# freshman97/LinTransUNet

Hardware: AMD Instinct MI355X
Metric: 128^3 CT patches/sec (fwd+bwd) (higher is better)
Workload: dtype bf16; 1 GPU; MaskTransUnet train step (fwd + 5-level loss + bwd), 128^3 single-channel patches, 2 per GPU, dropout 0.3, random-init weights; global_batch=2, parallelism=dp1, side_stream_concurrent=True, allreduce=none (1 rank)

## Files before the change

lintransunet_amd/csrc/linattn.hip:

```cpp
#include "common.h"

#define DK 32
#define TOK 32
#define PART_STRIDE (64 + 1024)
#ifndef LA_TR_PAD
#define LA_TR_PAD 32
#endif

__device__ __forceinline__ float xhalf_sum(float v) { return xhalf_combine<LtuAdd>(v); }
__device__ __forceinline__ float xhalf_max(float v) { return xhalf_combine<LtuMax>(v); }

__device__ __forceinline__ bf16x8 pack8(const float* v) {
  bf16x8 r;
#pragma unroll
  for (int e = 0; e < 8; ++e) r[e] = (__bf16)v[e];
  return r;
}
template <typename T>
struct IsBf16 { static constexpr bool value = false; };
template <>
struct IsBf16<bf16_t> { static constexpr bool value = true; };

template <typename T>
struct GVec;
// ... 401 lines not shown
      const float4 v = *reinterpret_cast<const float4*>(qrow + 4 * q4);
      a[4 * q4] = v.x; a[4 * q4 + 1] = v.y; a[4 * q4 + 2] = v.z; a[4 * q4 + 3] = v.w;
    }
    float mx = -INFINITY;
#pragma unroll
    for (int s = 0; s < 16; ++s) mx = fmaxf(mx, a[s]);
    mx = xhalf_max(mx);
    float sum = 0.f;
#pragma unroll
    for (int s = 0; s < 16; ++s) {
      a[s] = __expf(a[s] - mx);
      sum += a[s];
    }
    sum = xhalf_sum(sum);
    const float inv = rs / sum;
    if (lh == 0 && n0 + li < n_end) {
      float* qs = qstat + (((long long)b * N + n0 + li) * H + wave) * 2;
      qs[0] = mx;
      qs[1] = inv;
    }
    f32x16 acc;
#pragma unroll
    for (int r = 0; r < 16; ++r) acc[r] = 0.f;
    if constexpr (IsBf16<T>::value) {
#pragma unroll
      for (int s = 0; s < 16; ++s) a[s] *= inv;
      acc = __builtin_amdgcn_mfma_f32_32x32x16_bf16(pack8(a), cbb[0], acc, 0, 0, 0);
      acc = __builtin_amdgcn_mfma_f32_32x32x16_bf16(pack8(a + 8), cbb[1], acc, 0, 0, 0);
    } else {
#pragma unroll
      for (int s = 0; s < 16; ++s) acc = __builtin_amdgcn_mfma_f32_32x32x2f32(a[s] * inv, cb[s], acc, 0, 0, 0);
    }
    __syncthreads();
#pragma unroll
    for (int r = 0; r < 16; ++r) {
      const int t = (r & 3) + 8 * (r >> 2) + 4 * lh;
      smem[t * LDQ + wave * DK + li] = acc[r];
    }
    __syncthreads();
    constexpr int VPR = D / W;
#pragma unroll
    for (int p = 0; p < (TOK * VPR + NTHR - 1) / NTHR; ++p) {
      const int idx = tid + p * NTHR;
      const int t = idx / VPR, c = (idx % VPR) * W;
      if (idx < TOK * VPR && n0 + t < n_end) GVec<T>::from_lds(out + ((long long)b * N + n0 + t) * D + c, &smem[t * LDQ + c]);
    }
  }
}

#define LAW_HEADS 4
#define LAW_LD (LAW_HEADS * DK + 8)

template <int D>
__global__ void __launch_bounds__(256) linattn_apply_rows(const uint16_t* __restrict__ qkv, const float* __restrict__ ctx,
                                                         uint16_t* __restrict__ out, float* __restrict__ qstat, int N, int tiles_per_wave) {
  constexpr int H = D / DK, CG = H / LAW_HEADS;
  __shared__ __attribute__((aligned(16))) uint16_t smem[4 * TOK * LAW_LD];
  const int lane = threadIdx.x & 63, wave = threadIdx.x >> 6;
  const int li = lane & 31, lh = lane >> 5;
  uint16_t* tile = smem + wave * TOK * LAW_LD;
  const int b = blockIdx.y;
  const int gw = blockIdx.x * 4 + wave;
  const int cg = gw % CG;
  const int n_begin = (gw / CG) * tiles_per_wave * TOK;
  const int n_end = min(N, n_begin + tiles_per_wave * TOK);
  if (n_begin >= N) return;
  bf16x8 ca[LAW_HEADS][2];
#pragma unroll
  for (int hh = 0; hh < LAW_HEADS; ++hh) {
    const float* cx = ctx + ((long long)b * H + cg * LAW_HEADS + hh) * 1024;
#pragma unroll
    for (int u = 0; u < 2; ++u) {
      float t[8];
#pragma unroll
      for (int e = 0; e < 8; ++e) t[e] = cx[(16 * lh + 8 * u + e) * 32 + li];
      ca[hh][u] = pack8(t);
    }
  }
  const float rs = 0.17677669529663688110f;
  const int cr = lane >> 4, cc = (lane & 15) * 8;
  const uint16_t* qb = qkv + (long long)b * N * 3 * D + cg * (LAW_HEADS * DK) + cc;
  uint16_t* ob = out + (long long)b * N * D + cg * (LAW_HEADS * DK) + cc;
  uint4 nx[8];
  auto fetch = [&](int n0) {
#pragma unroll
    for (int p = 0; p < 8; ++p) {
      const int n = n0 + 4 * p + cr;
      nx[p] = make_uint4(0u, 0u, 0u, 0u);
      if (n < n_end) nx[p] = *reinterpret_cast<const uint4*>(qb + (long long)n * 3 * D);
    }
  };
  fetch(n_begin);
  for (int n0 = n_begin; n0 < n_end; n0 += TOK) {
#pragma unroll
    for (int p = 0; p < 8; ++p) *reinterpret_cast<uint4*>(tile + (4 * p + cr) * LAW_LD + cc) = nx[p];
    if (n0 + TOK < n_end) fetch(n0 + TOK);
    float2 st[LAW_HEADS];
#pragma unroll
    for (int hh = 0; hh < LAW_HEADS; ++hh) {
      const uint16_t* qr = tile + li * LAW_LD + hh * DK + 16 * lh;
      const uint4 v0 = *reinterpret_cast<const uint4*>(qr), v1 = *reinterpret_cast<const uint4*>(qr + 8);
      const uint32_t w[8] = {v0.x, v0.y, v0.z, v0.w, v1.x, v1.y, v1.z, v1.w};
      float a[16];
#pragma unroll
      for (int k = 0; k < 8; ++k) {
        a[2 * k] = __uint_as_float(w[k] << 16);
        a[2 * k + 1] = __uint_as_float(w[k] & 0xffff0000u);
      }
      float mx = a[0];
#pragma unroll
      for (int s = 1; s < 16; ++s) mx = fmaxf(mx, a[s]);
      mx = xhalf_max(mx);
      float sum = 0.f;
#pragma unroll
      for (int s = 0; s < 16; ++s) {
        a[s] = __expf(a[s] - mx);
        sum += a[s];
      }
      sum = xhalf_sum(sum);
      const float inv = rs / sum;
      st[hh] = make_float2(mx, inv);
#pragma unroll
      for (int s = 0; s < 16; ++s) a[s] *= inv;
      f32x16 acc;
#pragma unroll
      for (int r = 0; r < 16; ++r) acc[r] = 0.f;
      acc = __builtin_amdgcn_mfma_f32_32x32x16_bf16(ca[hh][0], pack8(a), acc, 0, 0, 0);
      acc = __builtin_amdgcn_mfma_f32_32x32x16_bf16(ca[hh][1], pack8(a + 8), acc, 0, 0, 0);
#pragma unroll
      for (int q = 0; q < 4; ++q) {
        uint2 v;
        v.x = pack_bf16x2(acc[4 * q], acc[4 * q + 1]);
        v.y = pack_bf16x2(acc[4 * q + 2], acc[4 * q + 3]);
        *reinterpret_cast<uint2*>(tile + li * LAW_LD + hh * DK + 8 * q + 4 * lh) = v;
      }
    }
    if (lh == 0 && n0 + li < n_end) {
      float4* qs = reinterpret_cast<float4*>(qstat + (((long long)b * N + n0 + li) * H + cg * LAW_HEADS) * 2);
      qs[0] = make_float4(st[0].x, st[0].y, st[1].x, st[1].y);
      qs[1] = make_float4(st[2].x, st[2].y, st[3].x, st[3].y);
    }
#pragma unroll
    for (int p = 0; p < 8; ++p) {
      const int n = n0 + 4 * p + cr;
      const uint4 v = *reinterpret_cast<const uint4*>(tile + (4 * p + cr) * LAW_LD + cc);
      if (n < n_end) *reinterpret_cast<uint4*>(ob + (long long)n * D) = v;
    }
  }
}

template <typename T, int D>
__global__ void __launch_bounds__(2 * D) linattn_dctx_partial(const T* __restrict__ qkv, const T* __restrict__ dout,
                                                             const float* __restrict__ qstat, float* __restrict__ part, int N,
                                                             int tokens_per_split) {
  constexpr int H = D / DK;
  extern __shared__ __attribute__((aligned(16))) float smem[];
  float* sq = smem;
  float* sg = smem + TOK * D;
  float* st = smem + 2 * TOK * D;
  const int b = blockIdx.y, sp = blockIdx.x, nsplit = gridDim.x;
  const int tid = threadIdx.x, lane = tid & 63, wave = tid >> 6;
  const int li = lane & 31, lh = lane >> 5;
  const int n_begin = sp * tokens_per_split;
  const int n_end = min(N, n_begin + tokens_per_split);
  const T* qb = qkv + (long long)b * N * 3 * D;
  const T* gb = dout + (long long)b * N * D;
  f32x16 acc;
#pragma unroll
  for (int r = 0; r < 16; ++r) acc[r] = 0.f;
  RowTile<T, D, D, D> tq, tg;
  static_assert(TOK * H * 2 <= 2 * D, "one statistics float per thread");
  auto load_stat = [&](int n0) {
    return (tid < TOK * H * 2 && n0 + tid / (H * 2) < n_end) ? qstat[((long long)b * N + n0) * H * 2 + tid] : 0.f;
  };
  if constexpr (IsBf16<T>::value) {
    constexpr int PQ = D + LA_TR_PAD;
    uint16_t* sm = reinterpret_cast<uint16_t*>(smem);
    float* stf = reinterpret_cast<float*>(sm + 4 * TOK * PQ);
    RowTile<T, D, D, PQ> bq, bg;
    const int off = tr_lane_offset(lane, PQ) + wave * DK;
    bq.load(qb, 3 * D, 0, n_begin, n_end, tid);
    bg.load(gb, D, 0, n_begin, n_end, tid);
    float stn = load_stat(n_begin);
    bq.store_raw(sm, tid);
    bg.store_raw(sm + TOK * PQ, tid);
    if (tid < TOK * H * 2) stf[tid] = stn;
    __syncthreads();
    int buf = 0;
    for (int n0 = n_begin; n0 < n_end; n0 += TOK) {
      const bool more = n0 + TOK < n_end;
      if (more) {
        bq.load(qb, 3 * D, 0, n0 + TOK, n_end, tid);
        bg.load(gb, D, 0, n0 + TOK, n_end, tid);
        stn = load_stat(n0 + TOK);
      }
      const uint16_t* S = sm + buf * (2 * TOK * PQ);
      const float* ST = stf + buf * (TOK * H * 2);
      const int ntok = min(TOK, n_end - n0);
#pragma unroll
      for (int u = 0; u < 2; ++u) {
        const bf16x8 qf = tr_frag(S + 16 * u * PQ + off, PQ), gf = tr_frag(S + (TOK + 16 * u) * PQ + off, PQ);
        float qe[8];
#pragma unroll
        for (int e = 0; e < 8; ++e) {
          const int t = 16 * u + 8 * lh + e;
          const float2 rs = *reinterpret_cast<const float2*>(ST + (t * H + wave) * 2);
          qe[e] = t < ntok ? __expf((float)qf[e] - rs.x) * rs.y : 0.f;
        }
        acc = __builtin_amdgcn_mfma_f32_32x32x16_bf16(gf, pack8(qe), acc, 0, 0, 0);
      }
      if (more) {
        uint16_t* Sn = sm + (buf ^ 1) * (2 * TOK * PQ);
        bq.store_raw(Sn, tid);
        bg.store_raw(Sn + TOK * PQ, tid);
        if (tid < TOK * H * 2) stf[(buf ^ 1) * (TOK * H * 2) + tid] = stn;
      }
      __syncthreads();
      buf ^= 1;
    }
  } else {
  tq.load(qb, 3 * D, 0, n_begin, n_end, tid);
  tg.load(gb, D, 0, n_begin, n_end, tid);
  float stn = load_stat(n_begin);
  for (int n0 = n_begin; n0 < n_end; n0 += TOK) {
    __syncthreads();
    tq.store(sq, tid);
    tg.store(sg, tid);
    if (tid < TOK * H * 2) st[tid] = stn;
    __syncthreads();
    if (n0 + TOK < n_end) {
      tq.load(qb, 3 * D, 0, n0 + TOK, n_end, tid);
      tg.load(gb, D, 0, n0 + TOK, n_end, tid);
      stn = load_stat(n0 + TOK);
    }
    const int ntok = min(TOK, n_end - n0);
    if constexpr (IsBf16<T>::value) {
#pragma unroll
      for (int u = 0; u < 2; ++u) {
        float qe[8], ge[8];
#pragma unroll
        for (int e = 0; e < 8; ++e) {
          const int t = 16 * u + 8 * lh + e;
          qe[e] = 0.f; ge[e] = 0.f;
          if (t < ntok) {
            qe[e] = __expf(sq[t * D + wave * DK + li] - st[(t * H + wave) * 2]) * st[(t * H + wave) * 2 + 1];
            ge[e] = sg[t * D + wave * DK + li];
          }
        }
        acc = __builtin_amdgcn_mfma_f32_32x32x16_bf16(pack8(ge), pack8(qe), acc, 0, 0, 0);
      }
    } else {
#pragma unroll
      for (int t0 = 0; t0 < TOK; t0 += 2) {
        const int t = t0 + lh;
        float qv = 0.f, gv = 0.f;
        if (t < ntok) {
          qv = __expf(sq[t * D + wave * DK + li] - st[(t * H + wave) * 2]) * st[(t * H + wave) * 2 + 1];
          gv = sg[t * D + wave * DK + li];
        }
        acc = __builtin_amdgcn_mfma_f32_32x32x2f32(gv, qv, acc, 0, 0, 0);
      }
    }
  }
  }
  float* out = part + (((long long)b * nsplit + sp) * H + wave) * 1024;
#pragma unroll
  for (int r = 0; r < 16; ++r) {
    const int j = (r & 3) + 8 * (r >> 2) + 4 * lh;
    out[j * 32 + li] = acc[r];
  }
}

template <int NB>
__global__ void __launch_bounds__(256) linattn_dctx_combine(const float* __restrict__ part, float* __restrict__ dctx, int nsplit, int H) {
  __shared__ float4 red4[7][32];
  const int bh = blockIdx.y, b = bh / H, h = bh % H;
  const float* p0 = part + ((long long)b * nsplit * H + h) * 1024 + blockIdx.x * 128;
  const int l = threadIdx.x & 31, grp = threadIdx.x >> 5;
  float4 a = make_float4(0.f, 0.f, 0.f, 0.f);
  for (int s0 = grp; s0 < nsplit; s0 += 8 * NB) {
    float4 v[NB];
#pragma unroll
    for (int k = 0; k < NB; ++k) {
      const int sp = s0 + 8 * k;
      v[k] = *reinterpret_cast<const float4*>(p0 + (long long)(sp < nsplit ? sp : s0) * H * 1024 + l * 4);
    }
#pragma unroll
    for (int k = 0; k < NB; ++k)
      if (s0 + 8 * k < nsplit) { a.x += v[k].x; a.y += v[k].y; a.z += v[k].z; a.w += v[k].w; }
  }
  if (grp > 0) red4[grp - 1][l] = a;
  __syncthreads();
  if (grp != 0) return;
#pragma unroll
  for (int q = 0; q < 7; ++q) {
    const float4 v = red4[q][l];
    a.x += v.x; a.y += v.y; a.z += v.z; a.w += v.w;
  }
  const int e = blockIdx.x * 128 + l * 4, jj = e >> 5, ii = e & 31;
  float* o = dctx + (long long)bh * 1024 + jj;
  o[ii * 32] = a.x; o[(ii + 1) * 32] = a.y; o[(ii + 2) * 32] = a.z; o[(ii + 3) * 32] = a.w;
}

template <typename T, int D>
__global__ void __launch_bounds__(2 * D, 2) linattn_bwd_apply(const T* __restrict__ qkv, const T* __restrict__ dout,
                                                          const float* __restrict__ ctx, const float* __restrict__ dctx,
                                                          const float* __restrict__ stats, const float* __restrict__ tvec,
                                                          const float* __restrict__ qstat, T* __restrict__ dqkv, int N, int tokb) {
  constexpr int H = D / DK, LD3 = 3 * D + 4, LD1 = D + 4, NTHR = 2 * D, W = GVec<T>::W;
  extern __shared__ __attribute__((aligned(16))) float smem[];
  const int b = blockIdx.y;
  const int tid = threadIdx.x, lane = tid & 63, wave = tid >> 6;
  const int li = lane & 31, lh = lane >> 5;
  float* gt = smem + TOK * LD3;
  float* cs = gt + TOK * LD1 + wave * 96;
  const long long bh = (long long)b * H + wave;
  if (lane < 32) {
    cs[lane] = stats[bh * 64 + lane];
    cs[32 + lane] = 1.f / stats[bh * 64 + 32 + lane];
  }
  float ctxA[16], dcA[16], dcT[16];
#pragma unroll
  for (int s = 0; s < 16; ++s) {
    ctxA[s] = ctx[bh * 1024 + li * 32 + 16 * lh + s];
    dcA[s] = dctx[bh * 1024 + li * 32 + 16 * lh + s];
    dcT[s] = dctx[bh * 1024 + (16 * lh + s) * 32 + li];
  }
  {
    float t = 0.f;
#pragma unroll
    for (int s = 0; s < 16; ++s) t += ctxA[s] * dcA[s];
    t = xhalf_sum(t);
    if (lane < 32) cs[64 + lane] = t;
  }
  const bf16x8 ctxB[2] = {pack8(ctxA), pack8(ctxA + 8)}, dcTB[2] = {pack8(dcT), pack8(dcT + 8)};
  bf16x8 dcAB[3][2];
  {
    float r1[16], r2[16];
#pragma unroll
    for (int s = 0; s < 16; ++s) {
      r1[s] = dcA[s] - (float)(__bf16)dcA[s];
      r2[s] = r1[s] - (float)(__bf16)r1[s];
    }
#pragma unroll
    for (int u = 0; u < 2; ++u) { dcAB[0][u] = pack8(dcA + 8 * u); dcAB[1][u] = pack8(r1 + 8 * u); dcAB[2][u] = pack8(r2 + 8 * u); }
  }
  const T* qb = qkv + (long long)b * N * 3 * D;
  const T* gb = dout + (long long)b * N * D;

  const int n_begin = blockIdx.x * tokb;
  const int n_end = min(N, n_begin + tokb);
  RowTile<T, D, 3 * D, LD3> tq;
  RowTile<T, D, D, LD1> tg;
  auto load_qs = [&](int n0) {
    return *reinterpret_cast<const float2*>(qstat + (((long long)b * N + min(n0 + li, n_end - 1)) * H + wave) * 2);
  };
  tq.load(qb, 3 * D, 0, n_begin, n_end, tid);
  tg.load(gb, D, 0, n_begin, n_end, tid);
  float2 qsn = load_qs(n_begin);
  tq.store(smem, tid);
  tg.store(gt, tid);
  __syncthreads();
  for (int n0 = n_begin; n0 < n_end; n0 += TOK) {
    const float rmax = qsn.x, rinv = qsn.y;
    const bool more = n0 + TOK < n_end;
    if (more) {
      tq.load(qb, 3 * D, 0, n0 + TOK, n_end, tid);
      tg.load(gb, D, 0, n0 + TOK, n_end, tid);
      qsn = load_qs(n0 + TOK);
    }
    const float* qrow = &smem[li * LD3 + wave * DK];
    const float* krow = qrow + D;
    const float* vrow = qrow + 2 * D;
    const float* grow = &gt[li * LD1 + wave * DK];

    float gj[16], kk[16], vj[16];
#pragma unroll
    for (int q4 = 0; q4 < 4; ++q4) {
      const float4 a = *reinterpret_cast<const float4*>(grow + 16 * lh + 4 * q4);
      const float4 c = *reinterpret_cast<const float4*>(krow + 16 * lh + 4 * q4);
      const float4 e = *reinterpret_cast<const float4*>(vrow + 16 * lh + 4 * q4);
      gj[4 * q4] = a.x; gj[4 * q4 + 1] = a.y; gj[4 * q4 + 2] = a.z; gj[4 * q4 + 3] = a.w;
      kk[4 * q4] = c.x; kk[4 * q4 + 1] = c.y; kk[4 * q4 + 2] = c.z; kk[4 * q4 + 3] = c.w;
      vj[4 * q4] = e.x; vj[4 * q4 + 1] = e.y; vj[4 * q4 + 2] = e.z; vj[4 * q4 + 3] = e.w;
    }
    f32x16 aq, av, ak;
#pragma unroll
    for (int r = 0; r < 16; ++r) { aq[r] = 0.f; av[r] = 0.f; ak[r] = 0.f; }
    if constexpr (IsBf16<T>::value) {
#pragma unroll
      for (int s = 0; s < 16; ++s) kk[s] = __expf(kk[s] - cs[16 * lh + s]) * cs[32 + 16 * lh + s];
#pragma unroll
      for (int u = 0; u < 2; ++u) {
        aq = __builtin_amdgcn_mfma_f32_32x32x16_bf16(ctxB[u], pack8(gj + 8 * u), aq, 0, 0, 0);
        av = __builtin_amdgcn_mfma_f32_32x32x16_bf16(dcTB[u], pack8(kk + 8 * u), av, 0, 0, 0);
        const bf16x8 vb = pack8(vj + 8 * u);
#pragma unroll
        for (int pc = 2; pc >= 0; --pc) ak = __builtin_amdgcn_mfma_f32_32x32x16_bf16(dcAB[pc][u], vb, ak, 0, 0, 0);
      }
    } else {
#pragma unroll
      for (int s = 0; s < 16; ++s) {
        const int ch = 16 * lh + s;
        const float pk = __expf(kk[s] - cs[ch]) * cs[32 + ch];
        aq = __builtin_amdgcn_mfma_f32_32x32x2f32(ctxA[s], gj[s], aq, 0, 0, 0);
        av = __builtin_amdgcn_mfma_f32_32x32x2f32(dcT[s], pk, av, 0, 0, 0);
        ak = __builtin_amdgcn_mfma_f32_32x32x2f32(dcA[s], vj[s], ak, 0, 0, 0);
      }
    }
    float dot = 0.f;
    float qsv[16], pkv[16];
#pragma unroll
    for (int g4 = 0; g4 < 4; ++g4) {
      const int i0 = 8 * g4 + 4 * lh;
      const float4 qv = *reinterpret_cast<const float4*>(qrow + i0);
      const float4 kv = *reinterpret_cast<const float4*>(krow + i0);
      const float qa[4] = {qv.x, qv.y, qv.z, qv.w}, ka[4] = {kv.x, kv.y, kv.z, kv.w};
#pragma unroll
      for (int e = 0; e < 4; ++e) {
        const int r = 4 * g4 + e;
        qsv[r] = __expf(qa[e] - rmax) * rinv;
        pkv[r] = __expf(ka[e] - cs[i0 + e]) * cs[32 + i0 + e];
        dot += qsv[r] * aq[r];
      }
    }
    dot = xhalf_sum(dot);
    dot *= 5.65685424949238019521f;
    __syncthreads();
#pragma unroll
    for (int g4 = 0; g4 < 4; ++g4) {
      const int i0 = 8 * g4 + 4 * lh;
      float4 oq, ok4, ov;
#pragma unroll
      for (int e = 0; e < 4; ++e) {
        const int r = 4 * g4 + e;
        f4at(oq, e) = qsv[r] * (aq[r] - dot);
        f4at(ok4, e) = pkv[r] * (ak[r] - cs[64 + i0 + e]);
        f4at(ov, e) = av[r];
      }
      *reinterpret_cast<float4*>(&smem[li * LD3 + wave * DK + i0]) = oq;
      *reinterpret_cast<float4*>(&smem[li * LD3 + D + wave * DK + i0]) = ok4;
      *reinterpret_cast<float4*>(&smem[li * LD3 + 2 * D + wave * DK + i0]) = ov;
    }
    __syncthreads();
    constexpr int VPR = 3 * D / W, NOUT = (TOK * VPR + NTHR - 1) / NTHR;
    typename GVec<T>::reg ovec[NOUT];
#pragma unroll
    for (int p = 0; p < NOUT; ++p) {
      const int idx = min(tid + p * NTHR, TOK * VPR - 1);
      ovec[p] = GVec<T>::pack_lds(&smem[(idx / VPR) * LD3 + (idx % VPR) * W]);
    }
    __syncthreads();
    if (more) {
      tq.store(smem, tid);
      tg.store(gt, tid);
    }
#pragma unroll
    for (int p = 0; p < NOUT; ++p) {
      const int idx = tid + p * NTHR;
      const int t = idx / VPR, c = (idx % VPR) * W;
      if (idx < TOK * VPR && n0 + t < n_end) GVec<T>::store_g(dqkv + ((long long)b * N + n0 + t) * 3 * D + c, ovec[p]);
    }
    __syncthreads();
  }
}

static int pick_splits(int B, int N, int d, int* tokens_per_split) {
  int total = -1;
  total = ltu_knob_pos("LTU_LA_SPLITS", d >= 256 ? 256 : 512);
  int want = total / (B > 0 ? B : 1);
  if (want < 1) want = 1;
  if (want > KVC_GROUP * KVC_GROUP) want = KVC_GROUP * KVC_GROUP;
  int tps = (N + want - 1) / want;
  tps = (tps + 31) / 32 * 32;
  if (tps < 32) tps = 32;
  *tokens_per_split = tps;
  return (N + tps - 1) / tps;
}
static int pick_tokb(int B, int N, int d) {
  const int blocks = ltu_knob_pos("LTU_LA_TOKB_BLOCKS", d <= 128 ? 512 : 256);
  long long per = ((long long)B * N + blocks - 1) / blocks;
  int tokb = (int)((per + 31) / 32 * 32);
  if (tokb < 32) tokb = 32;
  if (tokb > 512) tokb = 512;
  return tokb;
}

extern "C" int ltu_linattn_splits(int B, int N) {
  int tps;
  return pick_splits(B, N, 128, &tps);
}

#define LA_DISPATCH_D(d, ...)                                   \
  do {                                                          \
    if ((d) == 32) { constexpr int D = 32; __VA_ARGS__ }        \
    else if ((d) == 64) { constexpr int D = 64; __VA_ARGS__ }   \
    else if ((d) == 128) { constexpr int D = 128; __VA_ARGS__ } \
    else if ((d) == 256) { constexpr int D = 256; __VA_ARGS__ } \
    else return LTU_E_SHAPE;                                    \
  } while (0)

extern "C" int ltu_linattn_fwd(const void* qkv, void* out, float* ctx, float* colstats, float* qstat, float* part_ws,
                               long long ws_floats, int B, int N, int d, int dtype, ltu_stream_t s);
extern "C" long long ltu_linattn_ws_floats(int B, int N, int d) {
  int tps;
  const long long ns = pick_splits(B, N, d, &tps), H = d / 32;
  return (long long)B * (ns + (ns + KVC_GROUP - 1) / KVC_GROUP + 2) * H * PART_STRIDE;
}
extern "C" int ltu_linattn_ctx(const void* qkv, float* ctx, float* colstats, float* part_ws, long long ws_floats, int B, int N, int d,
                               int dtype, ltu_stream_t s) {
  return ltu_linattn_fwd(qkv, nullptr, ctx, colstats, nullptr, part_ws, ws_floats, B, N, d, dtype, s);
}
extern "C" int ltu_linattn_fwd(const void* qkv, void* out, float* ctx, float* colstats, float* qstat, float* part_ws,
                               long long ws_floats, int B, int N, int d, int dtype, ltu_stream_t s) {
  const int H = d / 32;
  int tps;
  const int nsplit = pick_splits(B, N, d, &tps);
  if ((long long)B * (nsplit + (nsplit + KVC_GROUP - 1) / KVC_GROUP + 2) * H * PART_STRIDE > ws_floats) return LTU_E_ARG;
  hipStream_t st = (hipStream_t)s;
  const int tokb = pick_tokb(B, N, d);
  LTU_DISPATCH_T(dtype, {
    LA_DISPATCH_D(d, {
      hipLaunchKernelGGL((linattn_kv_partial<T, D>), dim3(nsplit, B), dim3(2 * D), 0, st, (const T*)qkv, part_ws, N, tps);
      const int group = KVC_GROUP, ngroups = (nsplit + group - 1) / group;
      float* part2 = part_ws + (size_t)B * nsplit * H * PART_STRIDE;
      if (nsplit * 32 * sizeof(float) <= 48 * 1024 && !ltu_knob("LTU_LA_TWO_LEVEL", 0)) {
        const size_t fsb = (size_t)nsplit * 32 * sizeof(float);
        if (nsplit <= 32) hipLaunchKernelGGL(linattn_kv_combine1<4>, dim3(8, B * H), dim3(256), fsb, st, part_ws, nsplit, colstats, ctx, H);
        else if (nsplit <= 64) hipLaunchKernelGGL(linattn_kv_combine1<8>, dim3(8, B * H), dim3(256), fsb, st, part_ws, nsplit, colstats, ctx, H);
        else if (nsplit <= 128) hipLaunchKernelGGL(linattn_kv_combine1<16>, dim3(8, B * H), dim3(256), fsb, st, part_ws, nsplit, colstats, ctx, H);
        else hipLaunchKernelGGL(linattn_kv_combine1<32>, dim3(8, B * H), dim3(256), fsb, st, part_ws, nsplit, colstats, ctx, H);
      } else if (ngroups > 1) {
        hipLaunchKernelGGL(linattn_kv_combine, dim3(ngroups, B * H), dim3(1024), 0, st, part_ws, nsplit, group, part2, colstats, ctx, H, 0);
        hipLaunchKernelGGL(linattn_kv_combine, dim3(1, B * H), dim3(1024), 0, st, part2, ngroups, ngroups, nullptr, colstats, ctx, H, 1);
      } else {
        hipLaunchKernelGGL(linattn_kv_combine, dim3(1, B * H), dim3(1024), 0, st, part_ws, nsplit, nsplit, nullptr, colstats, ctx, H, 1);
      }
      if (out == nullptr) {
      } else if constexpr (IsBf16<T>::value && D >= 128) {
        constexpr int CG = D / DK / LAW_HEADS;
        const long long tiles = cdiv(N, TOK);
        long long tpw = cdiv((long long)B * tiles * CG, (long long)ltu_knob_pos("LTU_LA_APPLY_WAVES", 4096));
        if (tpw < 1) tpw = 1;
        const long long waves = cdiv(tiles, tpw) * CG;
        hipLaunchKernelGGL((linattn_apply_rows<D>), dim3((unsigned)cdiv(waves, 4), B), dim3(256), 0, st, (const uint16_t*)qkv, ctx, (uint16_t*)out, qstat, N, (int)tpw);
      } else {
        hipLaunchKernelGGL((linattn_apply<T, D>), dim3(cdiv(N, tokb), B), dim3(2 * D), 0, st, (const T*)qkv, ctx, (T*)out, qstat, N, tokb);
      }
    });
  });
  return ltu_check_launch();
}

extern "C" int ltu_linattn_bwd(const void* qkv, const void* dout, const float* ctx, const float* colstats,
                               const float* qstat, void* dqkv, float* dctx, float* tvec, float* part_ws, long long ws_floats, int B,
                               int N, int d, int dtype, ltu_stream_t s) {
  const int H = d / 32;
  int tps;
  const int nsplit = pick_splits(B, N, d, &tps);
  if ((long long)B * nsplit * H * 1024 > ws_floats) return LTU_E_ARG;
  hipStream_t st = (hipStream_t)s;
  const size_t lds_b = (size_t)(32 * (3 * d + 4) + 32 * (d + 4) + H * 96) * sizeof(float);
  const int tokb = pick_tokb(B, N, d);
  LTU_DISPATCH_T(dtype, {
    LA_DISPATCH_D(d, {
      const size_t lds_p = IsBf16<T>::value ? (size_t)4 * TOK * (D + LA_TR_PAD) * 2 + (size_t)2 * TOK * H * 2 * sizeof(float)
                                            : (size_t)(2 * TOK * D + TOK * H * 2) * sizeof(float);
      hipLaunchKernelGGL((linattn_dctx_partial<T, D>), dim3(nsplit, B), dim3(2 * D), lds_p, st, (const T*)qkv, (const T*)dout, qstat, part_ws, N, tps);
      if (nsplit <= 32) hipLaunchKernelGGL(linattn_dctx_combine<4>, dim3(8, B * H), dim3(256), 0, st, part_ws, dctx, nsplit, H);
      else if (nsplit <= 64) hipLaunchKernelGGL(linattn_dctx_combine<8>, dim3(8, B * H), dim3(256), 0, st, part_ws, dctx, nsplit, H);
      else if (nsplit <= 128) hipLaunchKernelGGL(linattn_dctx_combine<16>, dim3(8, B * H), dim3(256), 0, st, part_ws, dctx, nsplit, H);
      else hipLaunchKernelGGL(linattn_dctx_combine<32>, dim3(8, B * H), dim3(256), 0, st, part_ws, dctx, nsplit, H);
      hipLaunchKernelGGL((linattn_bwd_apply<T, D>), dim3(cdiv(N, tokb), B), dim3(2 * D), lds_b, st, (const T*)qkv, (const T*)dout, ctx, dctx, colstats, tvec, qstat, (T*)dqkv, N, tokb);
    });
  });
  return ltu_check_launch();
}
```

Before: 164.1 patches/s.

## Keep bf16 tiles in LDS for linear-attention backward apply and raise occupancy

The bf16 path of linattn_bwd_apply now keeps q/k/v/grad tiles in LDS as packed bf16 instead of widening them to fp32, which shrinks LDS per block and lets launch bounds request 4 blocks per SM instead of 2. It feeds MFMA operands straight from LDS, uses permlane32 swaps to reshuffle fragments, splits the three MFMA groups with sched barriers, and spills one ctx fragment to LDS to save registers. Results are written back in place as bf16 and copied out with 16-byte vector stores. The extra bit-twiddling and the higher register pressure from more resident blocks may offset some of the gain, and it only affects one backward kernel.

```diff
diff --git a/lintransunet_amd/csrc/linattn.hip b/lintransunet_amd/csrc/linattn.hip
--- a/lintransunet_amd/csrc/linattn.hip
+++ b/lintransunet_amd/csrc/linattn.hip
@@ -727,18 +727,31 @@
   o[ii * 32] = a.x; o[(ii + 1) * 32] = a.y; o[(ii + 2) * 32] = a.z; o[(ii + 3) * 32] = a.w;
 }
 
+typedef uint32_t la_u32x4 __attribute__((ext_vector_type(4)));
+typedef la_u32x4 __attribute__((may_alias)) la_lds16;
+typedef uint4 __attribute__((may_alias)) la_lds16w;
+typedef uint2 __attribute__((may_alias)) la_lds8;
+typedef bf16x8 __attribute__((may_alias)) la_ldsfrag;
+constexpr int LAB_PAD = 8;
+constexpr int LAB_OCC = 4;
+__device__ __forceinline__ void permlane32_swap(uint32_t& a, uint32_t& b) {
+  float fa = __uint_as_float(a), fb = __uint_as_float(b);
+  permlane32_swap(fa, fb);
+  a = __float_as_uint(fa); b = __float_as_uint(fb);
+}
 template <typename T, int D>
-__global__ void __launch_bounds__(2 * D, 2) linattn_bwd_apply(const T* __restrict__ qkv, const T* __restrict__ dout,
+__global__ void __launch_bounds__(2 * D, IsBf16<T>::value ? LAB_OCC : 2) linattn_bwd_apply(const T* __restrict__ qkv, const T* __restrict__ dout,
                                                           const float* __restrict__ ctx, const float* __restrict__ dctx,
                                                           const float* __restrict__ stats, const float* __restrict__ tvec,
                                                           const float* __restrict__ qstat, T* __restrict__ dqkv, int N, int tokb) {
   constexpr int H = D / DK, LD3 = 3 * D + 4, LD1 = D + 4, NTHR = 2 * D, W = GVec<T>::W;
+  constexpr int P4 = 4 * D + LAB_PAD;
   extern __shared__ __attribute__((aligned(16))) float smem[];
   const int b = blockIdx.y;
   const int tid = threadIdx.x, lane = tid & 63, wave = tid >> 6;
   const int li = lane & 31, lh = lane >> 5;
   float* gt = smem + TOK * LD3;
-  float* cs = gt + TOK * LD1 + wave * 96;
+  float* cs = (IsBf16<T>::value ? smem + TOK * P4 / 2 : gt + TOK * LD1) + wave * 96;
   const long long bh = (long long)b * H + wave;
   if (lane < 32) {
     cs[lane] = stats[bh * 64 + lane];
@@ -775,56 +788,182 @@
 
   const int n_begin = blockIdx.x * tokb;
   const int n_end = min(N, n_begin + tokb);
-  RowTile<T, D, 3 * D, LD3> tq;
-  RowTile<T, D, D, LD1> tg;
   auto load_qs = [&](int n0) {
     return *reinterpret_cast<const float2*>(qstat + (((long long)b * N + min(n0 + li, n_end - 1)) * H + wave) * 2);
   };
-  tq.load(qb, 3 * D, 0, n_begin, n_end, tid);
-  tg.load(gb, D, 0, n_begin, n_end, tid);
-  float2 qsn = load_qs(n_begin);
-  tq.store(smem, tid);
-  tg.store(gt, tid);
-  __syncthreads();
-  for (int n0 = n_begin; n0 < n_end; n0 += TOK) {
-    const float rmax = qsn.x, rinv = qsn.y;
-    const bool more = n0 + TOK < n_end;
-    if (more) {
-      tq.load(qb, 3 * D, 0, n0 + TOK, n_end, tid);
-      tg.load(gb, D, 0, n0 + TOK, n_end, tid);
-      qsn = load_qs(n0 + TOK);
-    }
-    const float* qrow = &smem[li * LD3 + wave * DK];
-    const float* krow = qrow + D;
-    const float* vrow = qrow + 2 * D;
-    const float* grow = &gt[li * LD1 + wave * DK];
-
-    float gj[16], kk[16], vj[16];
-#pragma unroll
-    for (int q4 = 0; q4 < 4; ++q4) {
-      const float4 a = *reinterpret_cast<const float4*>(grow + 16 * lh + 4 * q4);
-      const float4 c = *reinterpret_cast<const float4*>(krow + 16 * lh + 4 * q4);
-      const float4 e = *reinterpret_cast<const float4*>(vrow + 16 * lh + 4 * q4);
-      gj[4 * q4] = a.x; gj[4 * q4 + 1] = a.y; gj[4 * q4 + 2] = a.z; gj[4 * q4 + 3] = a.w;
-      kk[4 * q4] = c.x; kk[4 * q4 + 1] = c.y; kk[4 * q4 + 2] = c.z; kk[4 * q4 + 3] = c.w;
-      vj[4 * q4] = e.x; vj[4 * q4 + 1] = e.y; vj[4 * q4 + 2] = e.z; vj[4 * q4 + 3] = e.w;
-    }
-    f32x16 aq, av, ak;
-#pragma unroll
-    for (int r = 0; r < 16; ++r) { aq[r] = 0.f; av[r] = 0.f; ak[r] = 0.f; }
-    if constexpr (IsBf16<T>::value) {
-#pragma unroll
-      for (int s = 0; s < 16; ++s) kk[s] = __expf(kk[s] - cs[16 * lh + s]) * cs[32 + 16 * lh + s];
-#pragma unroll
-      for (int u = 0; u < 2; ++u) {
-        aq = __builtin_amdgcn_mfma_f32_32x32x16_bf16(ctxB[u], pack8(gj + 8 * u), aq, 0, 0, 0);
-        av = __builtin_amdgcn_mfma_f32_32x32x16_bf16(dcTB[u], pack8(kk + 8 * u), av, 0, 0, 0);
-        const bf16x8 vb = pack8(vj + 8 * u);
-#pragma unroll
-        for (int pc = 2; pc >= 0; --pc) ak = __builtin_amdgcn_mfma_f32_32x32x16_bf16(dcAB[pc][u], vb, ak, 0, 0, 0);
-      }
-    } else {
-#pragma unroll
+  if constexpr (IsBf16<T>::value) {
+    uint16_t* sm = reinterpret_cast<uint16_t*>(smem);
+    constexpr int VG = D / 8;
+    const int pr = tid / VG, pcol = (tid % VG) * 8;
+    const unsigned go3 = pr * 3 * D + pcol;
+    uint16_t* lq = sm + pr * P4 + pcol;
+    la_u32x4 rq[6], rg[2];
+    auto fetch = [&](int n0) {
+      const uint16_t* tqb = reinterpret_cast<const uint16_t*>(qb) + (long long)n0 * 3 * D;
+      const uint16_t* tgb = reinterpret_cast<const uint16_t*>(gb) + (long long)n0 * D;
+      const int last = n_end - n0 - 1;
+#pragma unroll
+      for (int h = 0; h < 2; ++h) {
+        const unsigned row = min(pr + 16 * h, last);
+#pragma unroll
+        for (int j = 0; j < 3; ++j) rq[3 * h + j] = *reinterpret_cast<const la_u32x4*>(tqb + row * 3 * D + pcol + j * D);
+        rg[h] = *reinterpret_cast<const la_u32x4*>(tgb + row * D + pcol);
+      }
+    };
+    auto to_lds = [&]() {
+#pragma unroll
+      for (int h = 0; h < 2; ++h) {
+#pragma unroll
+        for (int j = 0; j < 3; ++j) *reinterpret_cast<la_lds16*>(lq + 16 * h * P4 + j * D) = rq[3 * h + j];
+        *reinterpret_cast<la_lds16*>(lq + 16 * h * P4 + 3 * D) = rg[h];
+      }
+    };
+    auto load_qs16 = [&](int n0) {
+      const unsigned o = (unsigned)(min(li, n_end - 1 - n0) * H + wave) * 2;
+      return *reinterpret_cast<const float2*>(qstat + ((long long)b * N + n0) * H * 2 + o);
+    };
+    float2 qsn = load_qs16(n_begin);
+    fetch(n_begin);
+    to_lds();
+    asm volatile("" ::"v"(qsn.x), "v"(qsn.y));
+    __syncthreads();
+    la_ldsfrag* ctx0 = reinterpret_cast<la_ldsfrag*>(smem + TOK * P4 / 2 + H * 96) + tid;
+    *ctx0 = ctxB[0];
+    uint16_t* qrow = sm + li * P4 + wave * DK;
+    for (int n0 = n_begin; n0 < n_end; n0 += TOK) {
+      const float rmax = qsn.x, rinv = qsn.y;
+      const bool more = n0 + TOK < n_end;
+      if (more) fetch(n0 + TOK);
+      auto unpack = [](uint32_t w, float& lo, float& hi) { lo = __uint_as_float(w << 16); hi = __uint_as_float(w & 0xffff0000u); };
+      auto put_quad = [](uint16_t* dst, float a, float b, float c, float d) {
+        *reinterpret_cast<la_lds8*>(dst) = make_uint2(pack_bf16x2(a, b), pack_bf16x2(c, d));
+      };
+      {
+        f32x16 aq;
+#pragma unroll
+        for (int r = 0; r < 16; ++r) aq[r] = 0.f;
+#pragma unroll
+        for (int u = 0; u < 2; ++u)
+          aq = __builtin_amdgcn_mfma_f32_32x32x16_bf16(u == 0 ? *ctx0 : ctxB[1], *reinterpret_cast<const la_ldsfrag*>(qrow + 3 * D + 16 * lh + 8 * u), aq, 0, 0, 0);
+        uint4 q0 = *reinterpret_cast<const la_lds16w*>(qrow + 16 * lh), q1 = *reinterpret_cast<const la_lds16w*>(qrow + 16 * lh + 8);
+        permlane32_swap(q0.x, q0.z); permlane32_swap(q0.y, q0.w);
+        permlane32_swap(q1.x, q1.z); permlane32_swap(q1.y, q1.w);
+        const uint32_t qq[4][2] = {{q0.x, q0.y}, {q1.x, q1.y}, {q0.z, q0.w}, {q1.z, q1.w}};
+        float dot = 0.f;
+        float qsv[16];
+#pragma unroll
+        for (int g4 = 0; g4 < 4; ++g4) {
+          float qa[4];
+          unpack(qq[g4][0], qa[0], qa[1]);
+          unpack(qq[g4][1], qa[2], qa[3]);
+#pragma unroll
+          for (int e = 0; e < 4; ++e) {
+            const int r = 4 * g4 + e;
+            qsv[r] = __expf(qa[e] - rmax) * rinv;
+            dot += qsv[r] * aq[r];
+          }
+        }
+        dot = xhalf_sum(dot);
+        dot *= 5.65685424949238019521f;
+#pragma unroll
+        for (int g4 = 0; g4 < 4; ++g4)
+          put_quad(qrow + 8 * g4 + 4 * lh, qsv[4 * g4] * (aq[4 * g4] - dot), qsv[4 * g4 + 1] * (aq[4 * g4 + 1] - dot),
+                   qsv[4 * g4 + 2] * (aq[4 * g4 + 2] - dot), qsv[4 * g4 + 3] * (aq[4 * g4 + 3] - dot));
+      }
+      __builtin_amdgcn_sched_barrier(0);
+      if (more) qsn = load_qs16(n0 + TOK);
+      bf16x8 pb[2];
+      {
+        f32x16 ak;
+#pragma unroll
+        for (int r = 0; r < 16; ++r) ak[r] = 0.f;
+#pragma unroll
+        for (int u = 0; u < 2; ++u) {
+          const bf16x8 vf = *reinterpret_cast<const la_ldsfrag*>(qrow + 2 * D + 16 * lh + 8 * u);
+#pragma unroll
+          for (int pc = 2; pc >= 0; --pc) ak = __builtin_amdgcn_mfma_f32_32x32x16_bf16(dcAB[pc][u], vf, ak, 0, 0, 0);
+        }
+#pragma unroll
+        for (int u = 0; u < 2; ++u) {
+          const uint4 kw = *reinterpret_cast<const la_lds16w*>(qrow + D + 16 * lh + 8 * u);
+          float kk[8];
+          unpack(kw.x, kk[0], kk[1]);
+          unpack(kw.y, kk[2], kk[3]);
+          unpack(kw.z, kk[4], kk[5]);
+          unpack(kw.w, kk[6], kk[7]);
+#pragma unroll
+          for (int e = 0; e < 8; ++e) kk[e] = __expf(kk[e] - cs[16 * lh + 8 * u + e]) * cs[32 + 16 * lh + 8 * u + e];
+          pb[u] = pack8(kk);
+#pragma unroll
+          for (int e = 0; e < 4; ++e) permlane32_swap(kk[e], kk[4 + e]);
+#pragma unroll
+          for (int g = 0; g < 2; ++g) {
+            const int g4 = u + 2 * g, i0 = 8 * g4 + 4 * lh;
+            const float* pk = kk + 4 * g;
+            put_quad(qrow + D + i0, pk[0] * (ak[4 * g4] - cs[64 + i0]), pk[1] * (ak[4 * g4 + 1] - cs[64 + i0 + 1]),
+                     pk[2] * (ak[4 * g4 + 2] - cs[64 + i0 + 2]), pk[3] * (ak[4 * g4 + 3] - cs[64 + i0 + 3]));
+          }
+        }
+      }
+      __builtin_amdgcn_sched_barrier(0);
+      {
+        f32x16 av;
+#pragma unroll
+        for (int r = 0; r < 16; ++r) av[r] = 0.f;
+#pragma unroll
+        for (int u = 0; u < 2; ++u) av = __builtin_amdgcn_mfma_f32_32x32x16_bf16(dcTB[u], pb[u], av, 0, 0, 0);
+#pragma unroll
+        for (int g4 = 0; g4 < 4; ++g4)
+          put_quad(qrow + 2 * D + 8 * g4 + 4 * lh, av[4 * g4], av[4 * g4 + 1], av[4 * g4 + 2], av[4 * g4 + 3]);
+      }
+      __syncthreads();
+      la_u32x4 ovec[6];
+#pragma unroll
+      for (int p = 0; p < 6; ++p) ovec[p] = *reinterpret_cast<const la_lds16*>(lq + 16 * (p / 3) * P4 + (p % 3) * D);
+      if (more) to_lds();
+      asm volatile("" ::"v"(qsn.x), "v"(qsn.y));
+      uint16_t* ot = reinterpret_cast<uint16_t*>(dqkv) + ((long long)b * N + n0) * 3 * D;
+#pragma unroll
+      for (int p = 0; p < 6; ++p)
+        if (pr + 16 * (p / 3) < n_end - n0) *reinterpret_cast<la_u32x4*>(ot + 16 * (p / 3) * 3 * D + (p % 3) * D + go3) = ovec[p];
+      __syncthreads();
+    }
+  } else {
+    RowTile<T, D, 3 * D, LD3> tq;
+    RowTile<T, D, D, LD1> tg;
+    tq.load(qb, 3 * D, 0, n_begin, n_end, tid);
+    tg.load(gb, D, 0, n_begin, n_end, tid);
+    float2 qsn = load_qs(n_begin);
+    tq.store(smem, tid);
+    tg.store(gt, tid);
+    __syncthreads();
+    for (int n0 = n_begin; n0 < n_end; n0 += TOK) {
+      const float rmax = qsn.x, rinv = qsn.y;
+      const bool more = n0 + TOK < n_end;
+      if (more) {
+        tq.load(qb, 3 * D, 0, n0 + TOK, n_end, tid);
+        tg.load(gb, D, 0, n0 + TOK, n_end, tid);
+        qsn = load_qs(n0 + TOK);
+      }
+      const float* qrow = &smem[li * LD3 + wave * DK];
+      const float* krow = qrow + D;
+      const float* vrow = qrow + 2 * D;
+      const float* grow = &gt[li * LD1 + wave * DK];
+
+      float gj[16], kk[16], vj[16];
+  #pragma unroll
+      for (int q4 = 0; q4 < 4; ++q4) {
+        const float4 a = *reinterpret_cast<const float4*>(grow + 16 * lh + 4 * q4);
+        const float4 c = *reinterpret_cast<const float4*>(krow + 16 * lh + 4 * q4);
+        const float4 e = *reinterpret_cast<const float4*>(vrow + 16 * lh + 4 * q4);
+        gj[4 * q4] = a.x; gj[4 * q4 + 1] = a.y; gj[4 * q4 + 2] = a.z; gj[4 * q4 + 3] = a.w;
+        kk[4 * q4] = c.x; kk[4 * q4 + 1] = c.y; kk[4 * q4 + 2] = c.z; kk[4 * q4 + 3] = c.w;
+        vj[4 * q4] = e.x; vj[4 * q4 + 1] = e.y; vj[4 * q4 + 2] = e.z; vj[4 * q4 + 3] = e.w;
+      }
+      f32x16 aq, av, ak;
+  #pragma unroll
+      for (int r = 0; r < 16; ++r) { aq[r] = 0.f; av[r] = 0.f; ak[r] = 0.f; }
+  #pragma unroll
       for (int s = 0; s < 16; ++s) {
         const int ch = 16 * lh + s;
         const float pk = __expf(kk[s] - cs[ch]) * cs[32 + ch];
@@ -832,61 +971,61 @@
         av = __builtin_amdgcn_mfma_f32_32x32x2f32(dcT[s], pk, av, 0, 0, 0);
         ak = __builtin_amdgcn_mfma_f32_32x32x2f32(dcA[s], vj[s], ak, 0, 0, 0);
       }
-    }
-    float dot = 0.f;
-    float qsv[16], pkv[16];
-#pragma unroll
-    for (int g4 = 0; g4 < 4; ++g4) {
-      const int i0 = 8 * g4 + 4 * lh;
-      const float4 qv = *reinterpret_cast<const float4*>(qrow + i0);
-      const float4 kv = *reinterpret_cast<const float4*>(krow + i0);
-      const float qa[4] = {qv.x, qv.y, qv.z, qv.w}, ka[4] = {kv.x, kv.y, kv.z, kv.w};
-#pragma unroll
-      for (int e = 0; e < 4; ++e) {
-        const int r = 4 * g4 + e;
-        qsv[r] = __expf(qa[e] - rmax) * rinv;
-        pkv[r] = __expf(ka[e] - cs[i0 + e]) * cs[32 + i0 + e];
-        dot += qsv[r] * aq[r];
-      }
-    }
-    dot = xhalf_sum(dot);
-    dot *= 5.65685424949238019521f;
-    __syncthreads();
-#pragma unroll
-    for (int g4 = 0; g4 < 4; ++g4) {
-      const int i0 = 8 * g4 + 4 * lh;
-      float4 oq, ok4, ov;
-#pragma unroll
-      for (int e = 0; e < 4; ++e) {
-        const int r = 4 * g4 + e;
-        f4at(oq, e) = qsv[r] * (aq[r] - dot);
-        f4at(ok4, e) = pkv[r] * (ak[r] - cs[64 + i0 + e]);
-        f4at(ov, e) = av[r];
-      }
-      *reinterpret_cast<float4*>(&smem[li * LD3 + wave * DK + i0]) = oq;
-      *reinterpret_cast<float4*>(&smem[li * LD3 + D + wave * DK + i0]) = ok4;
-      *reinterpret_cast<float4*>(&smem[li * LD3 + 2 * D + wave * DK + i0]) = ov;
-    }
-    __syncthreads();
-    constexpr int VPR = 3 * D / W, NOUT = (TOK * VPR + NTHR - 1) / NTHR;
-    typename GVec<T>::reg ovec[NOUT];
-#pragma unroll
-    for (int p = 0; p < NOUT; ++p) {
-      const int idx = min(tid + p * NTHR, TOK * VPR - 1);
-      ovec[p] = GVec<T>::pack_lds(&smem[(idx / VPR) * LD3 + (idx % VPR) * W]);
-    }
-    __syncthreads();
-    if (more) {
-      tq.store(smem, tid);
-      tg.store(gt, tid);
-    }
-#pragma unroll
-    for (int p = 0; p < NOUT; ++p) {
-      const int idx = tid + p * NTHR;
-      const int t = idx / VPR, c = (idx % VPR) * W;
-      if (idx < TOK * VPR && n0 + t < n_end) GVec<T>::store_g(dqkv + ((long long)b * N + n0 + t) * 3 * D + c, ovec[p]);
-    }
-    __syncthreads();
+      float dot = 0.f;
+      float qsv[16], pkv[16];
+  #pragma unroll
+      for (int g4 = 0; g4 < 4; ++g4) {
+        const int i0 = 8 * g4 + 4 * lh;
+        const float4 qv = *reinterpret_cast<const float4*>(qrow + i0);
+        const float4 kv = *reinterpret_cast<const float4*>(krow + i0);
+        const float qa[4] = {qv.x, qv.y, qv.z, qv.w}, ka[4] = {kv.x, kv.y, kv.z, kv.w};
+  #pragma unroll
+        for (int e = 0; e < 4; ++e) {
+          const int r = 4 * g4 + e;
+          qsv[r] = __expf(qa[e] - rmax) * rinv;
+          pkv[r] = __expf(ka[e] - cs[i0 + e]) * cs[32 + i0 + e];
+          dot += qsv[r] * aq[r];
+        }
+      }
+      dot = xhalf_sum(dot);
+      dot *= 5.65685424949238019521f;
+      __syncthreads();
+  #pragma unroll
+      for (int g4 = 0; g4 < 4; ++g4) {
+        const int i0 = 8 * g4 + 4 * lh;
+        float4 oq, ok4, ov;
+  #pragma unroll
+        for (int e = 0; e < 4; ++e) {
+          const int r = 4 * g4 + e;
+          f4at(oq, e) = qsv[r] * (aq[r] - dot);
+          f4at(ok4, e) = pkv[r] * (ak[r] - cs[64 + i0 + e]);
+          f4at(ov, e) = av[r];
+        }
+        *reinterpret_cast<float4*>(&smem[li * LD3 + wave * DK + i0]) = oq;
+        *reinterpret_cast<float4*>(&smem[li * LD3 + D + wave * DK + i0]) = ok4;
+        *reinterpret_cast<float4*>(&smem[li * LD3 + 2 * D + wave * DK + i0]) = ov;
+      }
+      __syncthreads();
+      constexpr int VPR = 3 * D / W, NOUT = (TOK * VPR + NTHR - 1) / NTHR;
+      typename GVec<T>::reg ovec[NOUT];
+  #pragma unroll
+      for (int p = 0; p < NOUT; ++p) {
+        const int idx = min(tid + p * NTHR, TOK * VPR - 1);
+        ovec[p] = GVec<T>::pack_lds(&smem[(idx / VPR) * LD3 + (idx % VPR) * W]);
+      }
+      __syncthreads();
+      if (more) {
+        tq.store(smem, tid);
+        tg.store(gt, tid);
+      }
+  #pragma unroll
+      for (int p = 0; p < NOUT; ++p) {
+        const int idx = tid + p * NTHR;
+        const int t = idx / VPR, c = (idx % VPR) * W;
+        if (idx < TOK * VPR && n0 + t < n_end) GVec<T>::store_g(dqkv + ((long long)b * N + n0 + t) * 3 * D + c, ovec[p]);
+      }
+      __syncthreads();
+    }
   }
 }
 
@@ -985,7 +1124,8 @@
   const int nsplit = pick_splits(B, N, d, &tps);
   if ((long long)B * nsplit * H * 1024 > ws_floats) return LTU_E_ARG;
   hipStream_t st = (hipStream_t)s;
-  const size_t lds_b = (size_t)(32 * (3 * d + 4) + 32 * (d + 4) + H * 96) * sizeof(float);
+  const size_t lds_b = dtype == LTU_BF16 ? (size_t)TOK * (4 * d + LAB_PAD) * 2 + (size_t)H * 96 * sizeof(float) + (size_t)2 * d * 16
+                                         : (size_t)(32 * (3 * d + 4) + 32 * (d + 4) + H * 96) * sizeof(float);
   const int tokb = pick_tokb(B, N, d);
   LTU_DISPATCH_T(dtype, {
     LA_DISPATCH_D(d, {
```

Result: faster. 166.6 patches/s (median of 6 runs) (+1.5%).
